# KaHIP/KaMinPar

Hardware: NVIDIA H100
Metric: lp_edges_per_second (higher is better)
Workload: dtype int32

## Files before the change

kaminpar_b200/csrc/kmp_lp.cu:

```cuda
#include <cuda_runtime.h>

#include <algorithm>
#include <chrono>
#include <cstdio>
#include <cstring>
#include <new>
#include <string>
#include <vector>

#include <cstdlib>
#include <dlfcn.h>
#include <nccl.h>
#include <cub/device/device_radix_sort.cuh>
#include <cub/device/device_scan.cuh>

#include "../../include/kaminpar_b200_contraction.h"
#include "../../include/kaminpar_b200_lp.h"
#include "lp_commit.cuh"
#include "lp_device.cuh"
#include "lp_lowgroup.cuh"
#include "lp_strict.cuh"
#include "lp_sweep.cuh"

using namespace kmp;
// ... 109 lines not shown
  uint32_t num_isolated = 0;

  DevBuf<uint32_t> order;
  std::vector<uint32_t> list_off;
  uint32_t max_list = 0;
  uint32_t lists_S = 0, lists_G = 0, lists_thr = 0;
  int lists_seed = 0;
  bool lists_valid = false;

  DevBuf<uint32_t> label, favored, communities;
  DevBuf<int32_t> weight, maxw, minw;
  DevBuf<uint8_t> active;
  DevBuf<uint32_t> mv_u, mv_t, cslot, slotmap;
  DevBuf<uint8_t> acc;
  DevBuf<int32_t> incoming, chist, hist, jmin, out_cur, out_delta, ohist, ojmin;
  DevBuf<uint32_t> ctr32;
  DevBuf<unsigned long long> ctr64;
  DevBuf<uint32_t> t4_table_off, t4_item_entry, t4_item_chunk, t4_sel_entry, t4_sel_piece, t4_sel_begin;
  DevBuf<uint32_t> t4_item_u, t4_item_beg, t4_item_deg;
  std::vector<uint32_t> t4_item_off, t4_sel_off;
  struct HubWave {
    uint32_t item_lo, item_hi, sel_lo, sel_hi;
  };
  std::vector<HubWave> t4_waves;
  std::vector<uint32_t> t4_wave_off;
  uint64_t hub_wave_slots = 1ull << 28;
  DevBuf<Cand> t4_part_best, t4_part_fav;
  uint64_t t4_max_slots = 0;
  uint64_t t4_max_wave_edges = 0;
  uint32_t hub_bucket_cap = kBucketCap, hub_sel_limit = 0;
  DevBuf<unsigned long long> hub_tab;
  DevBuf<uint32_t> hub_cursor;
  DevBuf<HubOverflow> hub_ovf;
  uint32_t mover_cap = 0;
  uint32_t cur_subround = 0;
  uint32_t cur_sg = 0;
  DevBuf<uint8_t> sort_keys_in, sort_keys_out;
  DevBuf<uint32_t> sort_vals_in;
  DevBuf<unsigned char> cub_tmp;
  DevBuf<unsigned long long> pairs_a, pairs_b;
  DevBuf<int32_t> ct_vals_a, ct_vals_b;
  DevBuf<uint32_t> ct_flags, ct_rank, ct_cl;
  DevBuf<unsigned long long> ct_counter;
  bool slot_state_clean = false;

  bool graph_sorted = false;
  bool strict_seeded = false;
  DevBuf<int32_t> st_slot, st_ent_val, st_slot2, st_ent2_val, st_concurrent;
  DevBuf<uint32_t> st_ent_key, st_ent2_key, st_used, st_second, st_tie_best, st_tie_fav, st_chunks, st_sub_perm,
      st_match, st_buckets;
  DevBuf<kmp_strict::Rng> st_rng;
  DevBuf<kmp_strict::Stats> st_stats;

  uint32_t call_counter = 0;
  uint64_t kernel_launches = 0, sweep_launches = 0;
  uint32_t pull_rounds = 0, push_rounds = 0;
  uint32_t rank = 0, world = 1;
  ncclComm_t comm = nullptr;
  DevBuf<uint32_t> dist_send, dist_recv;
  uint32_t *direct_send = nullptr;
  uint32_t direct_cap = 0;
  DevBuf<unsigned> grid_bar;
  int fused_blocks = 0;
  int fused_blocks_refine = 0;
  uint32_t low_blocks[2][2][2] = {};
  uint32_t team_grid[2][2][2][4] = {};
// ... 311 lines not shown
  const uint64_t b = (threads_needed + block - 1) / block;
  return static_cast<uint32_t>(std::max<uint64_t>(1, std::min<uint64_t>(b, max_blocks)));
}
inline uint32_t capped(const kmp_lp_handle *h, uint32_t blocks) {
  return h->grid_cap != 0 && blocks > h->grid_cap ? h->grid_cap : blocks;
}

constexpr int team_size_index(int T) { return T == 32 ? 0 : T == 128 ? 1 : T == 512 ? 2 : 3; }
template <int SLOTS, int TEAMS, bool V16> constexpr size_t team_smem() {
  return static_cast<size_t>(SLOTS) * TEAMS * (V16 ? 6 : 8);
}

template <int MODE, bool EW, bool P64, int T, int SLOTS, int TEAMS, bool V16 = false>
void launch_team(kmp_lp_handle *h, const SweepArgs &a) {
  const uint32_t want = (a.list_size + TEAMS - 1) / TEAMS;
  const uint32_t blocks = capped(h, std::max<uint32_t>(1, std::min<uint32_t>(want, h->team_grid[MODE][EW][P64][team_size_index(T)])));
  sweep_team<MODE, EW, P64, T, SLOTS, TEAMS, V16><<<blocks, T * TEAMS, team_smem<SLOTS, TEAMS, V16>(), h->sweep_stream>>>(a);
}

template <int MODE, bool EW, bool P64, int T, int SLOTS, int TEAMS, bool V16 = false>
bool configure_team(kmp_lp_handle *h, int sms) {
  const auto kernel = sweep_team<MODE, EW, P64, T, SLOTS, TEAMS, V16>;
  constexpr size_t smem = team_smem<SLOTS, TEAMS, V16>();
  int per_sm = 0;
  if (cudaFuncSetAttribute(kernel, cudaFuncAttributeMaxDynamicSharedMemorySize, static_cast<int>(smem)) != cudaSuccess ||
      cudaOccupancyMaxActiveBlocksPerMultiprocessor(&per_sm, kernel, T * TEAMS, smem) != cudaSuccess || per_sm < 1) {
    return false;
  }
  h->team_grid[MODE][EW][P64][team_size_index(T)] = static_cast<uint32_t>(sms * per_sm);
  return true;
}

template <int MODE, bool EW, bool P64> bool configure_team_kernels(kmp_lp_handle *h, int sms) {
  cudaFuncSetAttribute(sweep_hub_scatter<MODE, EW, P64>, cudaFuncAttributeMaxDynamicSharedMemorySize, kHubScatterSmem);
  bool ok = configure_team<MODE, EW, P64, 32, 512, 8, !EW>(h, sms) && configure_team<MODE, EW, P64, 128, 2048, 4>(h, sms) &&
            configure_team<MODE, EW, P64, 512, 8192, 1>(h, sms);
  if constexpr (EW) {
    ok = ok && configure_team<MODE, EW, P64, 1024, 16384, 1>(h, sms);
  } else {
    ok = ok && configure_team<MODE, EW, P64, 1024, 32768, 1, true>(h, sms);
  }
  return ok;
}

template <int MODE, bool EW, bool P64> cudaError_t launch_sweep_t(kmp_lp_handle *h, int tier, const SweepArgs &a) {
  if (a.list_size == 0) {
    return cudaSuccess;
  }
  const uint32_t tgrid = capped(h, grid_for(a.list_size, 256));
  switch (tier) {
  case 0:
    sweep_thread<MODE, EW, P64, 8><<<tgrid, 256, 0, h->sweep_stream>>>(a);
    break;
  case 1:
    sweep_thread<MODE, EW, P64, 16><<<tgrid, 256, 0, h->sweep_stream>>>(a);
    break;
  case 2:
    sweep_thread<MODE, EW, P64, 32><<<tgrid, 256, 0, h->sweep_stream>>>(a);
    break;
  case 3:
    launch_team<MODE, EW, P64, 32, 512, 8, !EW>(h, a);
    break;
  case 4:
    launch_team<MODE, EW, P64, 128, 2048, 4>(h, a);
    break;
  case 5:
    launch_team<MODE, EW, P64, 512, 8192, 1>(h, a);
    break;
  case 6:
    if constexpr (EW) {
      launch_team<MODE, EW, P64, 1024, 16384, 1>(h, a);
    } else {
      launch_team<MODE, EW, P64, 1024, 32768, 1, true>(h, a);
    }
    break;
  default: {
    HubArgs hb{};
    const uint32_t s_idx = h->cur_subround;
    const uint32_t S = h->lists_S;
    const uint32_t first = h->list_off[kHubTier * S + s_idx] - h->list_off[kHubTier * S];
    hb.table_off = h->t4_table_off.p + first;
    hb.g_tab = h->hub_tab.p;
    hb.cursor = h->hub_cursor.p;
    hb.ovf = h->hub_ovf.p;
    hb.ovf_cap = static_cast<uint32_t>(std::min<uint64_t>(h->t4_max_wave_edges, 0xFFFFFFFFull));
    hb.bucket_cap = h->hub_bucket_cap;
    hb.sel_limit = h->hub_sel_limit;
    hb.stage_adjncy = h->adjncy_16b ? 1u : 0u;
    hb.rank = h->rank;
    hb.world = h->world;
    hb.sel_begin = h->t4_sel_begin.p + first;
    hb.hit = h->t4_hit.p + first;
    for (uint32_t w = h->t4_wave_off[s_idx]; w < h->t4_wave_off[s_idx + 1]; ++w) {
      const kmp_lp_handle::HubWave &wv = h->t4_waves[w];
      hb.item_entry = h->t4_item_entry.p + wv.item_lo;
      hb.item_chunk = h->t4_item_chunk.p + wv.item_lo;
      hb.item_u = h->t4_item_u.p + wv.item_lo;
      hb.item_beg = h->t4_item_beg.p + wv.item_lo;
      hb.item_deg = h->t4_item_deg.p + wv.item_lo;
      hb.num_items = wv.item_hi - wv.item_lo;
      hb.queue = h->ctr32.p + 64 + w;
      hb.ovf_count = h->ctr32.p + 512 + w;
      sweep_hub_scatter<MODE, EW, P64><<<capped(h, std::min<uint32_t>(hb.num_items, kSMs * 4)), kHubThreads, kHubScatterSmem, h->sweep_stream>>>(a, hb, h->m);
      hb.sel_entry = h->t4_sel_entry.p + wv.sel_lo;
      hb.sel_piece = h->t4_sel_piece.p + wv.sel_lo;
      hb.num_sel_items = wv.sel_hi - wv.sel_lo;
      hb.part_best = h->t4_part_best.p + (wv.sel_lo - h->t4_sel_off[s_idx]);
      hb.part_fav = h->t4_part_fav.p + (wv.sel_lo - h->t4_sel_off[s_idx]);
      sweep_hub_select<MODE><<<capped(h, std::min<uint32_t>((hb.num_sel_items + kSelWarps - 1) / kSelWarps, kSMs * 6)), kSelWarps * 32, 0, h->sweep_stream>>>(a, hb);
      h->kernel_launches += 2;
    }
    hb.part_best = h->t4_part_best.p;
    hb.part_fav = h->t4_part_fav.p;
    sweep_hub_final<MODE><<<capped(h, grid_for(static_cast<uint64_t>(a.list_size) * 32, 256)), 256, 0, h->sweep_stream>>>(a, hb);
    break;
  }
  }
  return cudaGetLastError();
}

int timed_begin(kmp_lp_handle *h, int tag, cudaStream_t st = nullptr) {
  if (!h->timing) {
    return -1;
  }
  if (st == nullptr) {
    st = h->stream;
  }
  if (h->sweep_events_used == h->sweep_events.size()) {
    cudaEvent_t x, y;
    cudaEventCreate(&x);
    cudaEventCreate(&y);
    h->sweep_events.emplace_back(x, y);
    h->sweep_event_group.push_back(0);
  }
  const int idx = static_cast<int>(h->sweep_events_used++);
  h->sweep_event_group[idx] = tag;
  cudaEventRecord(h->sweep_events[idx].first, st);
  return idx;
}
void timed_end(kmp_lp_handle *h, int idx, cudaStream_t st = nullptr) {
  if (idx >= 0) {
    cudaEventRecord(h->sweep_events[idx].second, st == nullptr ? h->stream : st);
  }
// ... 91 lines not shown
                                             h->sort_vals_in.p, h->order.p, static_cast<int>(n), 0, 8, h->stream));
  }
  std::vector<uint32_t> hist(512);
  KMP_CUDA(cudaMemcpyAsync(hist.data(), h->ctr32.p, 512 * sizeof(uint32_t), cudaMemcpyDeviceToHost, h->stream));
  KMP_CUDA(cudaStreamSynchronize(h->stream));
  tc.lap("lists: keys + sort (sync)");
  h->list_off.assign(nkeys + 1, 0);
  for (uint32_t kx = 0; kx < nkeys; ++kx) {
    h->list_off[kx + 1] = h->list_off[kx] + hist[kx];
  }
  auto lsize = [&](uint32_t tier, uint32_t sr) { return hist[tier * S + sr]; };
  h->max_list = 0;
  h->mover_cap = 1;
  for (uint32_t sr = 0; sr < S; ++sr) {
    for (int g = 0; g < kNumGroups; ++g) {
      uint32_t tot = 0;
      for (int t = first_tier_of_group(g); t <= last_tier_of_group(g); ++t) {
        tot += lsize(static_cast<uint32_t>(t), sr);
      }
      h->mover_cap = std::max(h->mover_cap, tot);
    }
  }
  KMP_CUDA(h->queue.ensure(static_cast<size_t>(kNumTiers) * kNumGroups * S));
  h->max_list = h->mover_cap;
  h->max_degree = hist[300];
  {
    const uint32_t t4_begin = h->list_off[kHubTier * S], t4_end = h->list_off[(kHubTier + 1) * S];
    const uint32_t t4_cnt = t4_end - t4_begin;
    h->t4_item_off.assign(S + 1, 0);
    h->t4_wave_off.assign(S + 1, 0);
    h->t4_waves.clear();
    h->t4_max_slots = 0;
    h->t4_max_wave_edges = 0;
    if (t4_cnt > 0) {
      DevBuf<uint32_t> &d_deg = h->t4_tmp_deg, &d_beg = h->t4_tmp_beg, &d_ids = h->t4_tmp_ids;
      KMP_CUDA(d_deg.ensure(t4_cnt));
      KMP_CUDA(d_beg.ensure(t4_cnt));
      KMP_CUDA(d_ids.ensure(t4_cnt));
      k_gather_degrees<<<grid_for(t4_cnt, 256), 256, 0, h->stream>>>(t4_cnt, h->order.p + t4_begin, h->xadj, d_deg.p,
                                                                      d_beg.p, d_ids.p);
      std::vector<uint32_t> vbeg(t4_cnt), vids(t4_cnt), iu, ibeg, ideg;
      KMP_CUDA(cudaMemcpyAsync(vbeg.data(), d_beg.p, t4_cnt * sizeof(uint32_t), cudaMemcpyDeviceToHost, h->stream));
      KMP_CUDA(cudaMemcpyAsync(vids.data(), d_ids.p, t4_cnt * sizeof(uint32_t), cudaMemcpyDeviceToHost, h->stream));
      std::vector<uint32_t> deg(t4_cnt), toff(t4_cnt), sbeg(t4_cnt), ient, ichk, sent, spiece;
      h->t4_sel_off.assign(S + 1, 0);
      size_t max_sel = 0;
      KMP_CUDA(cudaMemcpyAsync(deg.data(), d_deg.p, t4_cnt * sizeof(uint32_t), cudaMemcpyDeviceToHost, h->stream));
      KMP_CUDA(cudaStreamSynchronize(h->stream));
      uint64_t wave_slots = h->hub_wave_slots;
      {
        uint64_t total = 0;
        for (uint32_t i = 0; i < t4_cnt; ++i) {
          total += static_cast<uint64_t>(hub_buckets(deg[i])) * kBucketCap;
        }
        wave_slots = std::max<uint64_t>(wave_slots, total / (kMaxHubWaves / 2 - S) + 1);
      }
      for (uint32_t sr = 0; sr < S; ++sr) {
        const uint32_t lo = h->list_off[kHubTier * S + sr] - t4_begin, hi = h->list_off[kHubTier * S + sr + 1] - t4_begin;
        uint64_t slots = 0, wave_edges = 0;
        kmp_lp_handle::HubWave wave{static_cast<uint32_t>(ient.size()), 0, static_cast<uint32_t>(sent.size()), 0};
        auto close_wave = [&]() {
          wave.item_hi = static_cast<uint32_t>(ient.size());
          wave.sel_hi = static_cast<uint32_t>(sent.size());
          if (wave.item_hi > wave.item_lo) {
            h->t4_waves.push_back(wave);
          }
// ... 9 lines not shown
          const uint64_t cap = static_cast<uint64_t>(buckets) * kBucketCap;
          if (slots > 0 && slots + cap > wave_slots) {
            close_wave();
          }
          if ((slots + cap) / kBucketCap > 0xFFFFFFFFull) {
            return fail(KMP_ERR_UNSUPPORTED, "high-degree buckets of one wave exceed 2^32");
          }
          toff[i] = static_cast<uint32_t>(slots / kBucketCap);
          slots += cap;
          wave_edges += deg[i];
          const uint32_t chunks = (deg[i] + kChunkEdges - 1) / kChunkEdges;
          for (uint32_t c = 0; c < chunks; ++c) {
            ient.push_back(i - lo);
            ichk.push_back(c);
            iu.push_back(vids[i]);
            ibeg.push_back(vbeg[i]);
            ideg.push_back(deg[i]);
          }
          sbeg[i] = static_cast<uint32_t>(sent.size() - h->t4_sel_off[sr]);
          for (uint32_t c = 0; c < buckets; ++c) {
            sent.push_back(i - lo);
            spiece.push_back(c);
          }
        }
        close_wave();
        h->t4_wave_off[sr + 1] = static_cast<uint32_t>(h->t4_waves.size());
        h->t4_sel_off[sr + 1] = static_cast<uint32_t>(sent.size());
        max_sel = std::max<size_t>(max_sel, sent.size() - h->t4_sel_off[sr]);
        h->t4_item_off[sr + 1] = static_cast<uint32_t>(ient.size());
      }
      if (h->t4_waves.size() > kMaxHubWaves) {
        return fail(KMP_ERR_UNSUPPORTED, "too many high-degree table waves (raise KMP_HUB_WAVE_SLOTS)");
      }
      KMP_CUDA(h->t4_table_off.ensure(t4_cnt));
      KMP_CUDA(h->t4_hit.ensure(t4_cnt));
      KMP_CUDA(cudaMemsetAsync(h->t4_hit.p, 0, static_cast<size_t>(t4_cnt) * 4, h->stream));
      KMP_CUDA(h->t4_item_entry.ensure(ient.size()));
      KMP_CUDA(h->t4_item_chunk.ensure(ichk.size()));
      KMP_CUDA(cudaMemcpyAsync(h->t4_table_off.p, toff.data(), t4_cnt * 4, cudaMemcpyHostToDevice, h->stream));
      KMP_CUDA(cudaMemcpyAsync(h->t4_item_entry.p, ient.data(), ient.size() * 4, cudaMemcpyHostToDevice, h->stream));
      KMP_CUDA(cudaMemcpyAsync(h->t4_item_chunk.p, ichk.data(), ichk.size() * 4, cudaMemcpyHostToDevice, h->stream));
      KMP_CUDA(h->t4_item_u.ensure(iu.size()));
      KMP_CUDA(h->t4_item_beg.ensure(iu.size()));
      KMP_CUDA(h->t4_item_deg.ensure(iu.size()));
      KMP_CUDA(cudaMemcpyAsync(h->t4_item_u.p, iu.data(), iu.size() * 4, cudaMemcpyHostToDevice, h->stream));
      KMP_CUDA(cudaMemcpyAsync(h->t4_item_beg.p, ibeg.data(), iu.size() * 4, cudaMemcpyHostToDevice, h->stream));
      KMP_CUDA(cudaMemcpyAsync(h->t4_item_deg.p, ideg.data(), iu.size() * 4, cudaMemcpyHostToDevice, h->stream));
      KMP_CUDA(h->t4_sel_entry.ensure(sent.size()));
      KMP_CUDA(h->t4_sel_piece.ensure(spiece.size()));
      KMP_CUDA(h->t4_sel_begin.ensure(t4_cnt));
      KMP_CUDA(h->t4_part_best.ensure(max_sel));
      KMP_CUDA(h->t4_part_fav.ensure(max_sel));
      KMP_CUDA(cudaMemcpyAsync(h->t4_sel_entry.p, sent.data(), sent.size() * 4, cudaMemcpyHostToDevice, h->stream));
      KMP_CUDA(cudaMemcpyAsync(h->t4_sel_piece.p, spiece.data(), spiece.size() * 4, cudaMemcpyHostToDevice, h->stream));
      KMP_CUDA(cudaMemcpyAsync(h->t4_sel_begin.p, sbeg.data(), t4_cnt * 4, cudaMemcpyHostToDevice, h->stream));
      KMP_CUDA(cudaStreamSynchronize(h->stream));
    }
  }
  tc.lap("lists: hub metadata");
  h->lists_S = S;
  h->lists_G = h->cfg.sync_granule_log2;
  h->lists_thr = h->cfg.large_degree_threshold;
  h->lists_seed = h->cfg.seed;
  h->lists_valid = true;
  tc.lap("lists: done");
  return KMP_OK;
}

int ensure_scratch(kmp_lp_handle *h, int mode, uint32_t num_labels) {
  const size_t cap = std::max<uint32_t>(h->mover_cap, 1);
  KMP_CUDA(h->mv_u.ensure(cap));
  KMP_CUDA(h->mv_t.ensure(cap));
  KMP_CUDA(h->acc.ensure(cap));
  KMP_CUDA(h->ctr32.ensure(kCtr32Size));
  KMP_CUDA(h->ctr64.ensure(kCtrSize));
  KMP_CUDA(h->active.ensure(h->n));
  if (mode == 0) {
    KMP_CUDA(h->cslot.ensure(cap));
    const bool fresh = h->incoming.cap < h->n || h->slotmap.cap < h->n || h->chist.cap < cap * kLadderLevels;
    KMP_CUDA(h->incoming.ensure(h->n));
    KMP_CUDA(h->slotmap.ensure(h->n));
    KMP_CUDA(h->chist.ensure(cap * kLadderLevels));
    if (fresh || !h->slot_state_clean) {
      KMP_CUDA(cudaMemsetAsync(h->incoming.p, 0, h->incoming.cap * sizeof(int32_t), h->stream));
      KMP_CUDA(cudaMemsetAsync(h->slotmap.p, 0xFF, h->slotmap.cap * sizeof(uint32_t), h->stream));
      KMP_CUDA(cudaMemsetAsync(h->chist.p, 0, h->chist.cap * sizeof(int32_t), h->stream));
      h->slot_state_clean = true;
    }
  } else {
    const size_t kk = std::max<uint32_t>(num_labels, 1);
    KMP_CUDA(h->hist.ensure(kk * kLadderLevels));
    KMP_CUDA(h->ohist.ensure(kk * kLadderLevels));
    KMP_CUDA(h->jmin.ensure(kk));
    KMP_CUDA(h->ojmin.ensure(kk));
    KMP_CUDA(h->out_cur.ensure(kk));
    KMP_CUDA(h->out_delta.ensure(kk));
    KMP_CUDA(cudaMemsetAsync(h->hist.p, 0, kk * kLadderLevels * sizeof(int32_t), h->stream));
    KMP_CUDA(cudaMemsetAsync(h->ohist.p, 0, kk * kLadderLevels * sizeof(int32_t), h->stream));
  }
  if (h->t4_max_slots > 0) {
    KMP_CUDA(h->hub_tab.ensure(h->t4_max_slots));
    KMP_CUDA(h->hub_cursor.ensure(h->t4_max_slots / kBucketCap));
    KMP_CUDA(h->hub_ovf.ensure(std::max<uint64_t>(h->t4_max_wave_edges, 1)));
    KMP_CUDA(cudaGetLastError());
  }
  (void)num_labels;
  return KMP_OK;
}

struct RunCtx {
  int mode;
  uint32_t num_labels;
  int32_t max_cluster_weight;
  bool has_min;
  bool has_comm;
};

SweepArgs make_sweep_args(kmp_lp_handle *h, const RunCtx &rc) {
  SweepArgs a{};
  a.xadj = h->xadj;
  a.adjncy = h->adjncy;
  a.vwgt = h->vwgt;
  a.adjwgt = h->adjwgt;
  a.label = h->label.p;
  a.labg = h->labg.p;
  a.pull = false;
  a.window = make_window(0, 0);
  a.queue = h->queue.p;
  a.weight = h->weight.p;
  a.max_w = rc.mode == 1 ? h->maxw.p : nullptr;
  a.min_w = rc.has_min ? h->minw.p : nullptr;
  a.communities = rc.has_comm ? h->communities.p : nullptr;
  a.active = h->active.p;
// ... 1339 lines not shown
}

int kmp_lp_free_scratch(kmp_lp_handle *h) {
  if (h == nullptr) {
    return KMP_OK;
  }
  cudaSetDevice(h->device);
  cudaStreamSynchronize(h->stream);
  h->label.release();
  h->favored.release();
  h->communities.release();
  h->weight.release();
  h->maxw.release();
  h->minw.release();
  h->active.release();
  h->mv_u.release();
  h->mv_t.release();
  h->cslot.release();
  h->slotmap.release();
  h->acc.release();
  h->incoming.release();
  h->chist.release();
  h->hist.release();
  h->jmin.release();
  h->out_cur.release();
  h->out_delta.release();
  h->ohist.release();
  h->ojmin.release();
  h->ctr32.release();
  h->ctr64.release();
  h->hub_tab.release();
  h->hub_cursor.release();
  h->hub_ovf.release();
  h->labg.release();
  h->sort_keys_in.release();
  h->sort_keys_out.release();
  h->sort_vals_in.release();
  h->t4_tmp_deg.release();
  h->t4_tmp_beg.release();
  h->t4_tmp_ids.release();
  h->cub_tmp.release();
  h->pairs_a.release();
  h->pairs_b.release();
  h->ct_vals_a.release();
  h->ct_vals_b.release();
  h->ct_flags.release();
  h->ct_rank.release();
  h->ct_cl.release();
  h->ct_counter.release();
  for (DevBuf<uint32_t> *b : {&h->bal_cand, &h->bal_under, &h->bal_ctr32, &h->bal_target, &h->bal_lists, &h->bal_sv_a,
                              &h->bal_sv_b, &h->bal_blk}) {
    b->release();
  }
  for (DevBuf<int32_t> *b : {&h->bal_over, &h->bal_pbw, &h->bal_wt, &h->bal_prefix}) {
    b->release();
  }
  h->bal_flag.release();
  h->bal_key.release();
  h->bal_ctrl.release();
  h->bal_sk_a.release();
  h->bal_sk_b.release();
  h->ubal_deficit.release();
  h->ubal_tmask.release();
  {
    cudaMemPool_t pool = kmp_private_pool(h->device);
    if (pool != nullptr) {
// ... 304 lines not shown
```

kaminpar_b200/csrc/lp_sweep.cuh:

```cuda
#pragma once

#include "lp_device.cuh"
#include "lp_sortnet.cuh"

namespace kmp {

template <int MODE>
__device__ __forceinline__ void emit_proposal(const SweepArgs &a, uint32_t idx, uint32_t u, uint32_t target,
                                              int32_t uw) {
  a.mv_u[idx] = u;
  a.mv_t[idx] = target;
  if (!a.accumulate) {
    return;
  }
  if (MODE == 0) {
    atomicAdd(&a.incoming[target], uw);
  } else {
    const uint32_t lvl = ladder_level(bijective32(u, a.base_commit));
    atomicAdd(&a.hist[target * kLadderLevels + lvl], uw);
  }
}

__device__ __forceinline__ void block_count_flush(const SweepArgs &a, unsigned long long edges,
                                                  unsigned long long nodes) {
// ... 555 lines not shown

struct HubOverflow {
  uint32_t bucket;
  uint32_t key;
  int32_t rating;
  uint32_t pad;
};

struct HubArgs {
  const uint32_t *__restrict__ item_entry;
  const uint32_t *__restrict__ item_chunk;
  const uint32_t *__restrict__ item_u;
  const uint32_t *__restrict__ item_beg;
  const uint32_t *__restrict__ item_deg;
  uint32_t num_items;
  const uint32_t *__restrict__ table_off;
  unsigned long long *__restrict__ g_tab;
  uint32_t *__restrict__ cursor;
  HubOverflow *__restrict__ ovf;
  uint32_t *__restrict__ ovf_count;
  uint32_t ovf_cap;
  uint32_t bucket_cap;
  uint32_t sel_limit;
  uint32_t stage_adjncy;
  const uint32_t *__restrict__ sel_entry;
  const uint32_t *__restrict__ sel_piece;
  uint32_t num_sel_items;
  const uint32_t *__restrict__ sel_begin;
  Cand *__restrict__ part_best;
  Cand *__restrict__ part_fav;
  uint32_t rank, world;
  uint32_t *__restrict__ queue;
  uint32_t *__restrict__ hit;
};

__host__ __device__ __forceinline__ uint32_t hub_buckets(uint32_t full_degree) {
  const uint32_t need = (full_degree + kBucketTargetFill - 1) / kBucketTargetFill;
  uint32_t p = 1;
  while (p < need) {
    p <<= 1;
  }
  return p;
}

__device__ __forceinline__ uint32_t smem_u32(const void *p) {
  return static_cast<uint32_t>(__cvta_generic_to_shared(p));
}
__device__ __forceinline__ void mbar_init(uint64_t *bar, uint32_t count) {
  asm volatile("mbarrier.init.shared::cta.b64 [%0], %1;" ::"r"(smem_u32(bar)), "r"(count) : "memory");
}
__device__ __forceinline__ void mbar_arrive_expect_tx(uint64_t *bar, uint32_t bytes) {
  asm volatile("mbarrier.arrive.expect_tx.shared::cta.b64 _, [%0], %1;" ::"r"(smem_u32(bar)), "r"(bytes) : "memory");
}
__device__ __forceinline__ void mbar_wait(uint64_t *bar, uint32_t parity) {
  asm volatile(
      "{\n"
      ".reg .pred p;\n"
      "WAIT_LOOP:\n"
      "mbarrier.try_wait.parity.shared::cta.b64 p, [%0], %1;\n"
      "@p bra DONE;\n"
      "bra WAIT_LOOP;\n"
      "DONE:\n"
      "}\n" ::"r"(smem_u32(bar)),
      "r"(parity)
      : "memory");
}
// ... 180 lines not shown
          kk[j] = keys[s];
          rr[j] = vals[s];
          if (kk[j] != kEmpty) {
            keys[s] = kEmpty;
            vals[s] = 0;
          }
        }
#pragma unroll
        for (int j = 0; j < B; ++j) {
          bb[j] = bucket0 + (lowbias32(kk[j]) & pmask);
          pos[j] = kk[j] != kEmpty ? atomicAdd(&hb.cursor[bb[j]], 1u) : 0u;
        }
#pragma unroll
        for (int j = 0; j < B; ++j) {
          if (kk[j] != kEmpty) {
            if (pos[j] < hb.bucket_cap) {
              hb.g_tab[static_cast<size_t>(bb[j]) * kBucketCap + pos[j]] =
                  (static_cast<unsigned long long>(kk[j]) << 32) | static_cast<uint32_t>(rr[j]);
            } else {
              const uint32_t o = atomicAdd(hb.ovf_count, 1u);
              if (o < hb.ovf_cap) {
                hb.ovf[o] = HubOverflow{bb[j], kk[j], rr[j], 0u};
              }
            }
          }
        }
      }
      __syncwarp();
    }
  }
}

template <int MODE> __global__ void __launch_bounds__(kSelWarps * 32) sweep_hub_select(const SweepArgs a, const HubArgs hb) {
  __shared__ uint32_t s_keys[kSelWarps][kSelTableSlots];
  __shared__ int32_t s_vals[kSelWarps][kSelTableSlots];
  __shared__ uint32_t s_claims_all[kSelWarps];
  const int lane = threadIdx.x & 31;
  const int wib = threadIdx.x >> 5;
  uint32_t *keys = s_keys[wib];
  int32_t *vals = s_vals[wib];
  uint32_t *s_claims = &s_claims_all[wib];
  for (uint32_t s = lane; s < kSelTableSlots; s += 32) {
    keys[s] = kEmpty;
    vals[s] = 0;
  }
  if (lane == 0) {
    *s_claims = 0;
  }
  __syncwarp();
  const uint32_t nwarps = gridDim.x * kSelWarps;
  for (uint32_t it = blockIdx.x * kSelWarps + wib; it < hb.num_sel_items; it += nwarps) {
    const uint32_t entry = hb.sel_entry[it];
    const uint32_t u = a.list[entry];
    Cand c = cand_none(), f = cand_none();
    const bool act = (entry % hb.world == hb.rank) && (a.active == nullptr || a.pull || a.active[u] != 0);
    const uint32_t b = hb.table_off[entry] + hb.sel_piece[it];
    const uint32_t appended = act ? __ldcg(&hb.cursor[b]) : 0u;
    if (appended != 0) {
      const uint32_t full_deg = a.xadj[u + 1] - a.xadj[u];
      const uint32_t pbits = 31 - __clz(static_cast<int>(hub_buckets(full_deg)));
      const uint32_t own = a.label[u];
      const int32_t uw = a.vwgt != nullptr ? a.vwgt[u] : 1;
      const int32_t own_w = a.weight[own];
      const bool store_fav = (MODE == 0) && (uw == own_w) && (own_w <= a.max_cluster_weight / 2);
      const uint32_t n_reg = appended < hb.bucket_cap ? appended : hb.bucket_cap;
      const uint32_t n_ovf = appended > hb.bucket_cap ? min(__ldcg(hb.ovf_count), hb.ovf_cap) : 0u;
      uint32_t tcap = pow2_ceil(2 * appended);
      tcap = tcap < 64 ? 64u : tcap > kSelTableSlots ? kSelTableSlots : tcap;
      const uint32_t tmask = tcap - 1;
      const uint32_t full_limit = tcap / 2 + tcap / 8;
      const uint32_t limit = (hb.sel_limit != 0 && hb.sel_limit < full_limit) ? hb.sel_limit : full_limit;
      const unsigned long long *reg = hb.g_tab + static_cast<size_t>(b) * kBucketCap;
      auto insert = [&](uint32_t key, int32_t r) {
        uint32_t slot = lowbias32(key ^ 0x9E3779B9u) & tmask;
        while (true) {
          const uint32_t prev = atomicCAS(&keys[slot], kEmpty, key);
          if (prev == kEmpty) {
            atomicAdd(s_claims, 1u);
          }
          if (prev == kEmpty || prev == key) {
            atomicAdd(&vals[slot], r);
            return;
          }
          slot = (slot + 1) & tmask;
        }
      };
      uint32_t K = 1;
      while (true) {
        c = cand_none();
        f = cand_none();
        bool overflowed = false;
        for (uint32_t cls = 0; cls < K && !overflowed; ++cls) {
          constexpr int B = 4;
          for (uint32_t i0 = 0; i0 < n_reg && !overflowed; i0 += 32 * B) {
            unsigned long long e[B];
#pragma unroll
            for (int j = 0; j < B; ++j) {
              const uint32_t i = i0 + j * 32 + lane;
              e[j] = i < n_reg ? __ldcs(reg + i) : ~0ull;
            }
#pragma unroll
            for (int j = 0; j < B; ++j) {
              const uint32_t key = static_cast<uint32_t>(e[j] >> 32);
              if (key != kEmpty && ((lowbias32(key) >> pbits) & (K - 1)) == cls) {
                insert(key, static_cast<int32_t>(static_cast<uint32_t>(e[j])));
              }
            }
            if (n_ovf != 0) {
              __syncwarp();
              overflowed = *s_claims > limit;
              __syncwarp();
            }
          }
          for (uint32_t i0 = 0; i0 < n_ovf && !overflowed; i0 += 32 * B) {
#pragma unroll
            for (int j = 0; j < B; ++j) {
              const uint32_t i = i0 + j * 32 + lane;
              if (i < n_ovf) {
                const HubOverflow o = hb.ovf[i];
                if (o.bucket == b && ((lowbias32(o.key) >> pbits) & (K - 1)) == cls) {
                  insert(o.key, o.rating);
                }
              }
            }
            __syncwarp();
            overflowed = *s_claims > limit;
            __syncwarp();
          }
          __syncwarp();
          bool lazy_done = false;
          if (MODE == 0 && K == 1 && !overflowed) {
            Cand ct = cand_none();
            for (uint32_t s = lane; s < tcap; s += 32) {
              const uint32_t kx = keys[s];
              if (kx != kEmpty) {
                const int32_t r = vals[s];
                if (r >= ct.gain && r > 0) {
                  const Cand x{r, 0, tie_hash(a.base_tie, u, kx), kx};
                  if (cand_better<0>(x, ct)) {
                    ct = x;
                  }
                }
                if (store_fav && r >= f.gain && r > 0) {
                  const Cand y{r, 0, tie_hash(a.base_fav, u, kx), kx};
                  if (cand_better<0>(y, f)) {
                    f = y;
                  }
                }
              }
            }
            const Cand top = warp_argmax<0>(kFull, ct);
            bool top_ok = true;
            if (top.gain > 0) {
              top_ok = (a.weight[top.key] + uw <= a.max_cluster_weight) || (top.key == own);
              if (a.communities != nullptr) {
                top_ok = top_ok && (a.communities[top.key] == a.communities[own]);
              }
            }
            if (top_ok) {
              c = top;
              lazy_done = true;
            }
          }
          const bool evaluate = !overflowed && !lazy_done;
          for (uint32_t s0 = 0; s0 < tcap; s0 += 32 * B) {
            uint32_t kk[B];
            int32_t rr[B], ww[B];
#pragma unroll
            for (int j = 0; j < B; ++j) {
              const uint32_t s = s0 + j * 32 + lane;
              kk[j] = s < tcap ? keys[s] : kEmpty;
              rr[j] = kk[j] != kEmpty ? vals[s] : 0;
            }
#pragma unroll
            for (int j = 0; j < B; ++j) {
              ww[j] = (kk[j] != kEmpty && evaluate) ? a.weight[kk[j]] : 0;
            }
#pragma unroll
            for (int j = 0; j < B; ++j) {
              if (kk[j] != kEmpty) {
                const uint32_t s = s0 + j * 32 + lane;
                keys[s] = kEmpty;
                vals[s] = 0;
                if (evaluate) {
                  Cand ff;
                  const Cand cc = eval_candidate_w<MODE>(a, u, own, uw, own_w, kk[j], rr[j], ww[j],
                                                         store_fav && !(MODE == 0 && K == 1), ff);
                  if (cand_better<MODE>(cc, c)) {
                    c = cc;
                  }
                  if (MODE == 0 && cand_better<0>(ff, f)) {
                    f = ff;
                  }
                }
              }
            }
          }
          __syncwarp();
          if (lane == 0) {
            *s_claims = 0;
          }
          __syncwarp();
        }
        if (!overflowed) {
          break;
        }
        K <<= 1;
      }
      if (lane == 0) {
        hb.cursor[b] = 0;
      }
    }
    const Cand best = warp_argmax<MODE>(kFull, c);
    const Cand fav = (MODE == 0) ? warp_argmax<0>(kFull, f) : cand_none();
    if (lane == 0) {
      hb.part_best[it] = best;
      hb.part_fav[it] = fav;
    }
  }
}

template <int MODE> __global__ void __launch_bounds__(256) sweep_hub_final(const SweepArgs a, const HubArgs hb) {
  const int lane = threadIdx.x & 31;
  const uint32_t warp = (blockIdx.x * blockDim.x + threadIdx.x) >> 5;
  const uint32_t nwarps = (gridDim.x * blockDim.x) >> 5;
  unsigned long long edges = 0, nodes = 0;
  for (uint32_t i = warp; i < a.list_size; i += nwarps) {
    if (i % hb.world != hb.rank) {
      continue;
    }
    const uint32_t u = a.list[i];
    bool flag = true;
    if (a.active != nullptr) {
      int fl = 0, ht = 0;
      if (lane == 0) {
        fl = static_cast<int>(a.active[u]);
        if (a.pull) {
          ht = static_cast<int>(hb.hit[i]);
          hb.hit[i] = 0;
        }
      }
      fl = __shfl_sync(kFull, fl, 0);
      ht = __shfl_sync(kFull, ht, 0);
      flag = fl != 0;
      if (fl == 0 && ht == 0) {
        continue;
      }
    }
    const uint32_t full_deg = a.xadj[u + 1] - a.xadj[u];
    uint32_t deg = full_deg;
    if (deg > a.max_num_neighbors) {
      deg = a.max_num_neighbors;
    }
    const uint32_t own = a.label[u];
    const int32_t uw = a.vwgt != nullptr ? a.vwgt[u] : 1;
    const int32_t own_w = a.weight[own];
    const uint32_t pieces = hub_buckets(full_deg);
    const uint32_t first = hb.sel_begin[i];
    const bool store_fav = (MODE == 0) && (uw == own_w) && (own_w <= a.max_cluster_weight / 2);
    Cand c = cand_none(), f = cand_none();
    for (uint32_t q = lane; q < pieces; q += 32) {
      const Cand pb = hb.part_best[first + q];
      if (cand_better<MODE>(pb, c)) {
        c = pb;
      }
      if (MODE == 0) {
        const Cand pf = hb.part_fav[first + q];
        if (cand_better<0>(pf, f)) {
          f = pf;
        }
      }
    }
    const Cand best = warp_argmax<MODE>(kFull, c);
    const Cand fav = (MODE == 0) ? warp_argmax<0>(kFull, f) : cand_none();
    if (lane == 0) {
      edges += deg;
      nodes += 1;
      if (a.active != nullptr && flag) {
        a.active[u] = 0;
      }
      uint32_t target;
      if (finish_vertex<MODE>(a, u, own, store_fav, best, fav, target)) {
        const uint32_t idx = atomicAdd(a.mover_count, 1u);
        emit_proposal<MODE>(a, idx, u, target, uw);
      }
    }
  }
  block_count_flush(a, edges, nodes);
}

// ... 2 lines not shown
```

Before: 41.33 billion.

## Rate clusterer hub nodes via label gather and per-class shared-memory hashing

For the clustering mode, high-degree hub nodes are no longer scattered into global hash buckets and then selected per wave. Instead, one kernel gathers neighbor labels into a contiguous buffer. A 1024-thread block then rates each hash class of labels in a large shared-memory table, and splits the class further if the table overflows. Work items are ordered by descending degree. This removes the global atomic scatter, the bucket and overflow bookkeeping, and the per-wave launches. In exchange, every hub's degree is re-read once per class pass and an extra label buffer is allocated.

```diff
diff --git a/kaminpar_b200/csrc/kmp_lp.cu b/kaminpar_b200/csrc/kmp_lp.cu
--- a/kaminpar_b200/csrc/kmp_lp.cu
+++ b/kaminpar_b200/csrc/kmp_lp.cu
@@ -165,6 +165,10 @@
   DevBuf<unsigned long long> hub_tab;
   DevBuf<uint32_t> hub_cursor;
   DevBuf<HubOverflow> hub_ovf;
+  DevBuf<uint32_t> t4_lab_off, t4_rate_begin, t4_rate_entry, t4_rate_cls;
+  std::vector<uint32_t> t4_rate_off;
+  uint64_t t4_max_subround_edges = 0;
+  DevBuf<uint32_t> hub_lab;
   uint32_t mover_cap = 0;
   uint32_t cur_subround = 0;
   uint32_t cur_sg = 0;
@@ -542,7 +546,13 @@
 }
 
 template <int MODE, bool EW, bool P64> bool configure_team_kernels(kmp_lp_handle *h, int sms) {
-  cudaFuncSetAttribute(sweep_hub_scatter<MODE, EW, P64>, cudaFuncAttributeMaxDynamicSharedMemorySize, kHubScatterSmem);
+  if constexpr (MODE == 0) {
+    if (cudaFuncSetAttribute(sweep_hub_rate<EW>, cudaFuncAttributeMaxDynamicSharedMemorySize, rate_smem<EW>()) != cudaSuccess) {
+      return false;
+    }
+  } else {
+    cudaFuncSetAttribute(sweep_hub_scatter<MODE, EW, P64>, cudaFuncAttributeMaxDynamicSharedMemorySize, kHubScatterSmem);
+  }
   bool ok = configure_team<MODE, EW, P64, 32, 512, 8, !EW>(h, sms) && configure_team<MODE, EW, P64, 128, 2048, 4>(h, sms) &&
             configure_team<MODE, EW, P64, 512, 8192, 1>(h, sms);
   if constexpr (EW) {
@@ -589,36 +599,59 @@
     const uint32_t s_idx = h->cur_subround;
     const uint32_t S = h->lists_S;
     const uint32_t first = h->list_off[kHubTier * S + s_idx] - h->list_off[kHubTier * S];
-    hb.table_off = h->t4_table_off.p + first;
-    hb.g_tab = h->hub_tab.p;
-    hb.cursor = h->hub_cursor.p;
-    hb.ovf = h->hub_ovf.p;
-    hb.ovf_cap = static_cast<uint32_t>(std::min<uint64_t>(h->t4_max_wave_edges, 0xFFFFFFFFull));
-    hb.bucket_cap = h->hub_bucket_cap;
     hb.sel_limit = h->hub_sel_limit;
-    hb.stage_adjncy = h->adjncy_16b ? 1u : 0u;
     hb.rank = h->rank;
     hb.world = h->world;
-    hb.sel_begin = h->t4_sel_begin.p + first;
     hb.hit = h->t4_hit.p + first;
-    for (uint32_t w = h->t4_wave_off[s_idx]; w < h->t4_wave_off[s_idx + 1]; ++w) {
-      const kmp_lp_handle::HubWave &wv = h->t4_waves[w];
-      hb.item_entry = h->t4_item_entry.p + wv.item_lo;
-      hb.item_chunk = h->t4_item_chunk.p + wv.item_lo;
-      hb.item_u = h->t4_item_u.p + wv.item_lo;
-      hb.item_beg = h->t4_item_beg.p + wv.item_lo;
-      hb.item_deg = h->t4_item_deg.p + wv.item_lo;
-      hb.num_items = wv.item_hi - wv.item_lo;
-      hb.queue = h->ctr32.p + 64 + w;
-      hb.ovf_count = h->ctr32.p + 512 + w;
-      sweep_hub_scatter<MODE, EW, P64><<<capped(h, std::min<uint32_t>(hb.num_items, kSMs * 4)), kHubThreads, kHubScatterSmem, h->sweep_stream>>>(a, hb, h->m);
-      hb.sel_entry = h->t4_sel_entry.p + wv.sel_lo;
-      hb.sel_piece = h->t4_sel_piece.p + wv.sel_lo;
-      hb.num_sel_items = wv.sel_hi - wv.sel_lo;
-      hb.part_best = h->t4_part_best.p + (wv.sel_lo - h->t4_sel_off[s_idx]);
-      hb.part_fav = h->t4_part_fav.p + (wv.sel_lo - h->t4_sel_off[s_idx]);
-      sweep_hub_select<MODE><<<capped(h, std::min<uint32_t>((hb.num_sel_items + kSelWarps - 1) / kSelWarps, kSMs * 6)), kSelWarps * 32, 0, h->sweep_stream>>>(a, hb);
+    if constexpr (MODE == 0) {
+      const uint32_t ilo = h->t4_item_off[s_idx], ihi = h->t4_item_off[s_idx + 1];
+      hb.item_entry = h->t4_item_entry.p + ilo;
+      hb.item_chunk = h->t4_item_chunk.p + ilo;
+      hb.item_u = h->t4_item_u.p + ilo;
+      hb.item_beg = h->t4_item_beg.p + ilo;
+      hb.item_deg = h->t4_item_deg.p + ilo;
+      hb.num_items = ihi - ilo;
+      hb.lab = h->hub_lab.p;
+      hb.lab_off = h->t4_lab_off.p + first;
+      sweep_hub_gather<P64><<<capped(h, std::min<uint32_t>(hb.num_items, kSMs * 8)), 256, 0, h->sweep_stream>>>(a, hb);
+      const uint32_t rlo = h->t4_rate_off[s_idx], rhi = h->t4_rate_off[s_idx + 1];
+      hb.item_entry = h->t4_rate_entry.p + rlo;
+      hb.item_cls = h->t4_rate_cls.p + rlo;
+      hb.num_items = rhi - rlo;
+      hb.sel_begin = h->t4_rate_begin.p + first;
+      hb.part_best = h->t4_part_best.p;
+      hb.part_fav = h->t4_part_fav.p;
+      hb.queue = h->ctr32.p + 64 + s_idx;
+      sweep_hub_rate<EW><<<capped(h, std::min<uint32_t>(hb.num_items, kSMs)), kRateThreads, rate_smem<EW>(), h->sweep_stream>>>(a, hb);
       h->kernel_launches += 2;
+    } else {
+      hb.table_off = h->t4_table_off.p + first;
+      hb.g_tab = h->hub_tab.p;
+      hb.cursor = h->hub_cursor.p;
+      hb.ovf = h->hub_ovf.p;
+      hb.ovf_cap = static_cast<uint32_t>(std::min<uint64_t>(h->t4_max_wave_edges, 0xFFFFFFFFull));
+      hb.bucket_cap = h->hub_bucket_cap;
+      hb.stage_adjncy = h->adjncy_16b ? 1u : 0u;
+      hb.sel_begin = h->t4_sel_begin.p + first;
+      for (uint32_t w = h->t4_wave_off[s_idx]; w < h->t4_wave_off[s_idx + 1]; ++w) {
+        const kmp_lp_handle::HubWave &wv = h->t4_waves[w];
+        hb.item_entry = h->t4_item_entry.p + wv.item_lo;
+        hb.item_chunk = h->t4_item_chunk.p + wv.item_lo;
+        hb.item_u = h->t4_item_u.p + wv.item_lo;
+        hb.item_beg = h->t4_item_beg.p + wv.item_lo;
+        hb.item_deg = h->t4_item_deg.p + wv.item_lo;
+        hb.num_items = wv.item_hi - wv.item_lo;
+        hb.queue = h->ctr32.p + 64 + w;
+        hb.ovf_count = h->ctr32.p + 512 + w;
+        sweep_hub_scatter<MODE, EW, P64><<<capped(h, std::min<uint32_t>(hb.num_items, kSMs * 4)), kHubThreads, kHubScatterSmem, h->sweep_stream>>>(a, hb, h->m);
+        hb.sel_entry = h->t4_sel_entry.p + wv.sel_lo;
+        hb.sel_piece = h->t4_sel_piece.p + wv.sel_lo;
+        hb.num_sel_items = wv.sel_hi - wv.sel_lo;
+        hb.part_best = h->t4_part_best.p + (wv.sel_lo - h->t4_sel_off[s_idx]);
+        hb.part_fav = h->t4_part_fav.p + (wv.sel_lo - h->t4_sel_off[s_idx]);
+        sweep_hub_select<MODE><<<capped(h, std::min<uint32_t>((hb.num_sel_items + kSelWarps - 1) / kSelWarps, kSMs * 6)), kSelWarps * 32, 0, h->sweep_stream>>>(a, hb);
+        h->kernel_launches += 2;
+      }
     }
     hb.part_best = h->t4_part_best.p;
     hb.part_fav = h->t4_part_fav.p;
@@ -776,6 +809,7 @@
     h->t4_waves.clear();
     h->t4_max_slots = 0;
     h->t4_max_wave_edges = 0;
+    h->t4_max_subround_edges = 0;
     if (t4_cnt > 0) {
       DevBuf<uint32_t> &d_deg = h->t4_tmp_deg, &d_beg = h->t4_tmp_beg, &d_ids = h->t4_tmp_ids;
       KMP_CUDA(d_deg.ensure(t4_cnt));
@@ -851,6 +885,41 @@
       if (h->t4_waves.size() > kMaxHubWaves) {
         return fail(KMP_ERR_UNSUPPORTED, "too many high-degree table waves (raise KMP_HUB_WAVE_SLOTS)");
       }
+      std::vector<uint32_t> loff(t4_cnt), rbeg(t4_cnt), rent, rcls, ord;
+      h->t4_rate_off.assign(S + 1, 0);
+      size_t max_rate = 0;
+      for (uint32_t sr = 0; sr < S; ++sr) {
+        const uint32_t lo = h->list_off[kHubTier * S + sr] - t4_begin, hi = h->list_off[kHubTier * S + sr + 1] - t4_begin;
+        uint64_t edges = 0;
+        uint32_t res = 0;
+        ord.clear();
+        for (uint32_t i = lo; i < hi; ++i) {
+          loff[i] = static_cast<uint32_t>(edges);
+          edges += deg[i];
+          rbeg[i] = res;
+          res += hub_classes(deg[i]);
+          ord.push_back(i);
+        }
+        std::stable_sort(ord.begin(), ord.end(), [&](uint32_t x, uint32_t y) { return deg[x] > deg[y]; });
+        for (const uint32_t i : ord) {
+          for (uint32_t c = 0; c < hub_classes(deg[i]); ++c) {
+            rent.push_back(i - lo);
+            rcls.push_back(c);
+          }
+        }
+        h->t4_rate_off[sr + 1] = static_cast<uint32_t>(rent.size());
+        max_rate = std::max<size_t>(max_rate, res);
+        h->t4_max_subround_edges = std::max(h->t4_max_subround_edges, edges);
+      }
+      max_sel = std::max(max_sel, max_rate);
+      KMP_CUDA(h->t4_lab_off.ensure(t4_cnt));
+      KMP_CUDA(h->t4_rate_begin.ensure(t4_cnt));
+      KMP_CUDA(h->t4_rate_entry.ensure(rent.size()));
+      KMP_CUDA(h->t4_rate_cls.ensure(rcls.size()));
+      KMP_CUDA(cudaMemcpyAsync(h->t4_lab_off.p, loff.data(), t4_cnt * 4, cudaMemcpyHostToDevice, h->stream));
+      KMP_CUDA(cudaMemcpyAsync(h->t4_rate_begin.p, rbeg.data(), t4_cnt * 4, cudaMemcpyHostToDevice, h->stream));
+      KMP_CUDA(cudaMemcpyAsync(h->t4_rate_entry.p, rent.data(), rent.size() * 4, cudaMemcpyHostToDevice, h->stream));
+      KMP_CUDA(cudaMemcpyAsync(h->t4_rate_cls.p, rcls.data(), rcls.size() * 4, cudaMemcpyHostToDevice, h->stream));
       KMP_CUDA(h->t4_table_off.ensure(t4_cnt));
       KMP_CUDA(h->t4_hit.ensure(t4_cnt));
       KMP_CUDA(cudaMemsetAsync(h->t4_hit.p, 0, static_cast<size_t>(t4_cnt) * 4, h->stream));
@@ -917,7 +986,10 @@
     KMP_CUDA(cudaMemsetAsync(h->hist.p, 0, kk * kLadderLevels * sizeof(int32_t), h->stream));
     KMP_CUDA(cudaMemsetAsync(h->ohist.p, 0, kk * kLadderLevels * sizeof(int32_t), h->stream));
   }
-  if (h->t4_max_slots > 0) {
+  if (mode == 0 && h->t4_max_subround_edges > 0) {
+    KMP_CUDA(h->hub_lab.ensure(h->t4_max_subround_edges));
+  }
+  if (mode == 1 && h->t4_max_slots > 0) {
     KMP_CUDA(h->hub_tab.ensure(h->t4_max_slots));
     KMP_CUDA(h->hub_cursor.ensure(h->t4_max_slots / kBucketCap));
     KMP_CUDA(h->hub_ovf.ensure(std::max<uint64_t>(h->t4_max_wave_edges, 1)));
@@ -2323,6 +2395,7 @@
   h->hub_tab.release();
   h->hub_cursor.release();
   h->hub_ovf.release();
+  h->hub_lab.release();
   h->labg.release();
   h->sort_keys_in.release();
   h->sort_keys_out.release();
diff --git a/kaminpar_b200/csrc/lp_sweep.cuh b/kaminpar_b200/csrc/lp_sweep.cuh
--- a/kaminpar_b200/csrc/lp_sweep.cuh
+++ b/kaminpar_b200/csrc/lp_sweep.cuh
@@ -611,6 +611,9 @@
   uint32_t rank, world;
   uint32_t *__restrict__ queue;
   uint32_t *__restrict__ hit;
+  uint32_t *__restrict__ lab;
+  const uint32_t *__restrict__ lab_off;
+  const uint32_t *__restrict__ item_cls;
 };
 
 __host__ __device__ __forceinline__ uint32_t hub_buckets(uint32_t full_degree) {
@@ -857,6 +860,7 @@
 }
 
 template <int MODE> __global__ void __launch_bounds__(kSelWarps * 32) sweep_hub_select(const SweepArgs a, const HubArgs hb) {
+  static_assert(MODE == 1, "the clusterer rates its hubs with sweep_hub_rate");
   __shared__ uint32_t s_keys[kSelWarps][kSelTableSlots];
   __shared__ int32_t s_vals[kSelWarps][kSelTableSlots];
   __shared__ uint32_t s_claims_all[kSelWarps];
@@ -877,7 +881,7 @@
   for (uint32_t it = blockIdx.x * kSelWarps + wib; it < hb.num_sel_items; it += nwarps) {
     const uint32_t entry = hb.sel_entry[it];
     const uint32_t u = a.list[entry];
-    Cand c = cand_none(), f = cand_none();
+    Cand c = cand_none();
     const bool act = (entry % hb.world == hb.rank) && (a.active == nullptr || a.pull || a.active[u] != 0);
     const uint32_t b = hb.table_off[entry] + hb.sel_piece[it];
     const uint32_t appended = act ? __ldcg(&hb.cursor[b]) : 0u;
@@ -887,7 +891,6 @@
       const uint32_t own = a.label[u];
       const int32_t uw = a.vwgt != nullptr ? a.vwgt[u] : 1;
       const int32_t own_w = a.weight[own];
-      const bool store_fav = (MODE == 0) && (uw == own_w) && (own_w <= a.max_cluster_weight / 2);
       const uint32_t n_reg = appended < hb.bucket_cap ? appended : hb.bucket_cap;
       const uint32_t n_ovf = appended > hb.bucket_cap ? min(__ldcg(hb.ovf_count), hb.ovf_cap) : 0u;
       uint32_t tcap = pow2_ceil(2 * appended);
@@ -913,7 +916,6 @@
       uint32_t K = 1;
       while (true) {
         c = cand_none();
-        f = cand_none();
         bool overflowed = false;
         for (uint32_t cls = 0; cls < K && !overflowed; ++cls) {
           constexpr int B = 4;
@@ -953,41 +955,7 @@
             __syncwarp();
           }
           __syncwarp();
-          bool lazy_done = false;
-          if (MODE == 0 && K == 1 && !overflowed) {
-            Cand ct = cand_none();
-            for (uint32_t s = lane; s < tcap; s += 32) {
-              const uint32_t kx = keys[s];
-              if (kx != kEmpty) {
-                const int32_t r = vals[s];
-                if (r >= ct.gain && r > 0) {
-                  const Cand x{r, 0, tie_hash(a.base_tie, u, kx), kx};
-                  if (cand_better<0>(x, ct)) {
-                    ct = x;
-                  }
-                }
-                if (store_fav && r >= f.gain && r > 0) {
-                  const Cand y{r, 0, tie_hash(a.base_fav, u, kx), kx};
-                  if (cand_better<0>(y, f)) {
-                    f = y;
-                  }
-                }
-              }
-            }
-            const Cand top = warp_argmax<0>(kFull, ct);
-            bool top_ok = true;
-            if (top.gain > 0) {
-              top_ok = (a.weight[top.key] + uw <= a.max_cluster_weight) || (top.key == own);
-              if (a.communities != nullptr) {
-                top_ok = top_ok && (a.communities[top.key] == a.communities[own]);
-              }
-            }
-            if (top_ok) {
-              c = top;
-              lazy_done = true;
-            }
-          }
-          const bool evaluate = !overflowed && !lazy_done;
+          const bool evaluate = !overflowed;
           for (uint32_t s0 = 0; s0 < tcap; s0 += 32 * B) {
             uint32_t kk[B];
             int32_t rr[B], ww[B];
@@ -1009,13 +977,9 @@
                 vals[s] = 0;
                 if (evaluate) {
                   Cand ff;
-                  const Cand cc = eval_candidate_w<MODE>(a, u, own, uw, own_w, kk[j], rr[j], ww[j],
-                                                         store_fav && !(MODE == 0 && K == 1), ff);
-                  if (cand_better<MODE>(cc, c)) {
+                  const Cand cc = eval_candidate_w<1>(a, u, own, uw, own_w, kk[j], rr[j], ww[j], false, ff);
+                  if (cand_better<1>(cc, c)) {
                     c = cc;
-                  }
-                  if (MODE == 0 && cand_better<0>(ff, f)) {
-                    f = ff;
                   }
                 }
               }
@@ -1036,12 +1000,298 @@
         hb.cursor[b] = 0;
       }
     }
-    const Cand best = warp_argmax<MODE>(kFull, c);
-    const Cand fav = (MODE == 0) ? warp_argmax<0>(kFull, f) : cand_none();
+    const Cand best = warp_argmax<1>(kFull, c);
     if (lane == 0) {
       hb.part_best[it] = best;
-      hb.part_fav[it] = fav;
-    }
+    }
+  }
+}
+
+constexpr int kRateThreads = 1024;
+constexpr uint32_t kRateSlots = 16384;
+constexpr uint32_t kRateListCap = kRateSlots / 2;
+constexpr uint32_t kHubClassEdges = 8192;
+constexpr uint32_t kRateStage = 64;
+template <bool EW> constexpr int rate_smem() {
+  return static_cast<int>(kRateSlots * 8 + kRateListCap * 2 + (kRateThreads / 32) * kRateStage * (EW ? 8 : 4));
+}
+
+__host__ __device__ __forceinline__ uint32_t hub_classes(uint32_t full_degree) {
+  const uint32_t need = (full_degree + kHubClassEdges - 1) / kHubClassEdges;
+  uint32_t p = 1;
+  while (p < need) {
+    p <<= 1;
+  }
+  return p;
+}
+
+template <bool P64> __global__ void __launch_bounds__(256) sweep_hub_gather(const SweepArgs a, const HubArgs hb) {
+  constexpr int B = kChunkEdges / 256;
+  const int lane = threadIdx.x & 31;
+  for (uint32_t it = blockIdx.x; it < hb.num_items; it += gridDim.x) {
+    const uint32_t entry = hb.item_entry[it];
+    const uint32_t u = hb.item_u[it];
+    if (entry % hb.world != hb.rank || !(a.active == nullptr || a.pull || a.active[u] != 0)) {
+      continue;
+    }
+    const uint32_t deg = min(hb.item_deg[it], a.max_num_neighbors);
+    const uint32_t cbeg = hb.item_chunk[it] * kChunkEdges;
+    if (cbeg >= deg) {
+      continue;
+    }
+    const uint32_t cend = min(cbeg + kChunkEdges, deg);
+    const uint32_t *adj = a.adjncy + hb.item_beg[it];
+    uint32_t *out = hb.lab + hb.lab_off[entry];
+    uint32_t v[B];
+#pragma unroll
+    for (int j = 0; j < B; ++j) {
+      const uint32_t e = cbeg + j * 256 + threadIdx.x;
+      v[j] = e < cend ? adj[e] : kEmpty;
+    }
+    bool hit = false;
+#pragma unroll
+    for (int j = 0; j < B; ++j) {
+      if (v[j] != kEmpty) {
+        const typename LabG<P64>::word g = load_labg<P64>(a, v[j]);
+        hit = hit || stamp_hit(LabG<P64>::stamp(g), a.window);
+        out[cbeg + j * 256 + threadIdx.x] = LabG<P64>::label(g);
+      }
+    }
+    if (a.pull && __any_sync(kFull, hit) && lane == 0) {
+      atomicOr(&hb.hit[entry], 1u);
+    }
+  }
+}
+
+template <bool EW>
+__device__ __forceinline__ bool rate_insert(uint32_t *keys, int32_t *vals, uint16_t *list, uint32_t *s_claims,
+                                            uint32_t limit, uint32_t key, int32_t w, bool valid, int lane) {
+  uint32_t slot = 0;
+  bool claimed = false;
+  if (valid) {
+    slot = lowbias32(key ^ 0x9E3779B9u) & (kRateSlots - 1);
+    while (true) {
+      const uint32_t prev = atomicCAS(&keys[slot], kEmpty, key);
+      if (prev == kEmpty || prev == key) {
+        claimed = prev == kEmpty;
+        if (EW || !claimed) {
+          atomicAdd(&vals[slot], w);
+        }
+        break;
+      }
+      slot = (slot + 1) & (kRateSlots - 1);
+    }
+  }
+  const unsigned mask = __ballot_sync(kFull, claimed);
+  if (mask == 0) {
+    return false;
+  }
+  const uint32_t n = __popc(mask);
+  uint32_t base = 0;
+  if (lane == 0) {
+    base = atomicAdd(s_claims, n);
+  }
+  base = __shfl_sync(kFull, base, 0);
+  const uint32_t idx = base + __popc(mask & ((1u << lane) - 1u));
+  if (claimed && idx < kRateListCap) {
+    list[idx] = static_cast<uint16_t>(slot);
+  }
+  return base + n > limit;
+}
+
+template <bool EW> __global__ void __launch_bounds__(kRateThreads, 1) sweep_hub_rate(const SweepArgs a, const HubArgs hb) {
+  constexpr int T = kRateThreads;
+  constexpr int kWarps = T / 32;
+  constexpr int B = 8;
+  extern __shared__ __align__(16) unsigned char smem_raw[];
+  uint32_t *keys = reinterpret_cast<uint32_t *>(smem_raw);
+  int32_t *vals = reinterpret_cast<int32_t *>(smem_raw + sizeof(uint32_t) * kRateSlots);
+  uint32_t *stage_k = reinterpret_cast<uint32_t *>(smem_raw + 8 * kRateSlots);
+  int32_t *stage_w = reinterpret_cast<int32_t *>(stage_k + kWarps * kRateStage);
+  uint16_t *list = reinterpret_cast<uint16_t *>(stage_k + (EW ? 2 : 1) * kWarps * kRateStage);
+  __shared__ Cand s_red[kWarps];
+  __shared__ uint32_t s_item, s_claims;
+  const int tid = threadIdx.x;
+  const int lane = tid & 31;
+  const int wib = tid >> 5;
+  const unsigned below = (1u << lane) - 1u;
+  uint32_t *stk = stage_k + wib * kRateStage;
+  int32_t *stw = stage_w + wib * kRateStage;
+  for (uint32_t s = tid; s < kRateSlots; s += T) {
+    keys[s] = kEmpty;
+    vals[s] = 0;
+  }
+  const uint32_t limit = (hb.sel_limit != 0 && hb.sel_limit < kRateListCap) ? max(hb.sel_limit, 2u) : kRateListCap;
+  while (true) {
+    if (tid == 0) {
+      s_item = atomicAdd(hb.queue, 1u);
+    }
+    __syncthreads();
+    const uint32_t it = s_item;
+    if (it >= hb.num_items) {
+      break;
+    }
+    const uint32_t entry = hb.item_entry[it];
+    const uint32_t c0 = hb.item_cls[it];
+    const uint32_t u = a.list[entry];
+    if (entry % hb.world == hb.rank && (a.active == nullptr || a.pull || a.active[u] != 0)) {
+      const uint32_t beg = a.xadj[u];
+      const uint32_t full_deg = a.xadj[u + 1] - beg;
+      const uint32_t deg = min(full_deg, a.max_num_neighbors);
+      const uint32_t K0 = hub_classes(full_deg);
+      const uint32_t own = a.label[u];
+      const int32_t uw = a.vwgt != nullptr ? a.vwgt[u] : 1;
+      const int32_t own_w = a.weight[own];
+      const bool store_fav = (uw == own_w) && (own_w <= a.max_cluster_weight / 2);
+      const uint32_t *lab = hb.lab + hb.lab_off[entry];
+      Cand best = cand_none(), fav = cand_none();
+      uint32_t cls = c0, K = K0;
+      while (true) {
+        if (tid == 0) {
+          s_claims = 0;
+        }
+        __syncthreads();
+        bool wover = false;
+        uint32_t head = 0, pend = 0;
+        for (uint32_t e0 = wib * 32 * B; e0 < deg && !wover; e0 += T * B) {
+          uint32_t kb[B];
+#pragma unroll
+          for (int j = 0; j < B; ++j) {
+            const uint32_t e = e0 + j * 32 + lane;
+            kb[j] = e < deg ? __ldcg(lab + e) : kEmpty;
+          }
+#pragma unroll
+          for (int j = 0; j < B; ++j) {
+            if (!wover) {
+              const bool in = kb[j] != kEmpty && (lowbias32(kb[j]) & (K - 1)) == cls;
+              const unsigned m = __ballot_sync(kFull, in);
+              if (in) {
+                const uint32_t pos = (head + pend + __popc(m & below)) & (kRateStage - 1);
+                stk[pos] = kb[j];
+                if (EW) {
+                  stw[pos] = a.adjwgt[beg + e0 + j * 32 + lane];
+                }
+              }
+              pend += __popc(m);
+              if (pend >= 32) {
+                __syncwarp();
+                const uint32_t sl = (head + lane) & (kRateStage - 1);
+                wover = rate_insert<EW>(keys, vals, list, &s_claims, limit, stk[sl], EW ? stw[sl] : 1, true, lane);
+                __syncwarp();
+                head = (head + 32) & (kRateStage - 1);
+                pend -= 32;
+              }
+            }
+          }
+        }
+        if (!wover) {
+          __syncwarp();
+          const bool v = lane < pend;
+          const uint32_t sl = (head + lane) & (kRateStage - 1);
+          wover = rate_insert<EW>(keys, vals, list, &s_claims, limit, v ? stk[sl] : 0u, (EW && v) ? stw[sl] : 1, v, lane);
+        }
+        const bool over = __syncthreads_or(wover);
+        if (over) {
+          for (uint32_t s = tid; s < kRateSlots; s += T) {
+            keys[s] = kEmpty;
+            vals[s] = 0;
+          }
+          K <<= 1;
+          __syncthreads();
+          continue;
+        }
+        const uint32_t nc = s_claims;
+        Cand c = cand_none(), f = cand_none();
+        for (uint32_t l = tid; l < nc; l += T) {
+          const uint32_t s = list[l];
+          const uint32_t k = keys[s];
+          const int32_t r = vals[s] + (EW ? 0 : 1);
+          if (r > 0 && r >= c.gain) {
+            const Cand x{r, 0, tie_hash(a.base_tie, u, k), k};
+            if (cand_better<0>(x, c)) {
+              c = x;
+            }
+          }
+          if (store_fav && r > 0 && r >= f.gain) {
+            const Cand y{r, 0, tie_hash(a.base_fav, u, k), k};
+            if (cand_better<0>(y, f)) {
+              f = y;
+            }
+          }
+        }
+        Cand cb = team_argmax<0, T>(1, tid, c, s_red);
+        if (store_fav) {
+          const Cand cf = team_argmax<0, T>(1, tid, f, s_red);
+          if (cand_better<0>(cf, fav)) {
+            fav = cf;
+          }
+        }
+        bool top_ok = true;
+        if (cb.gain > 0) {
+          top_ok = (a.weight[cb.key] + uw <= a.max_cluster_weight) || (cb.key == own);
+          if (a.communities != nullptr) {
+            top_ok = top_ok && (a.communities[cb.key] == a.communities[own]);
+          }
+        }
+        if (!top_ok) {
+          Cand ce = cand_none();
+          for (uint32_t l0 = 0; l0 < nc; l0 += T * 4) {
+            uint32_t kk[4];
+            int32_t rr[4], ww[4];
+#pragma unroll
+            for (int j = 0; j < 4; ++j) {
+              const uint32_t l = l0 + j * T + tid;
+              const uint32_t s = l < nc ? list[l] : 0u;
+              kk[j] = l < nc ? keys[s] : kEmpty;
+              rr[j] = l < nc ? vals[s] + (EW ? 0 : 1) : 0;
+            }
+#pragma unroll
+            for (int j = 0; j < 4; ++j) {
+              ww[j] = kk[j] != kEmpty ? a.weight[kk[j]] : 0;
+            }
+#pragma unroll
+            for (int j = 0; j < 4; ++j) {
+              if (kk[j] != kEmpty) {
+                Cand ff;
+                const Cand cc = eval_candidate_w<0>(a, u, own, uw, own_w, kk[j], rr[j], ww[j], false, ff);
+                if (cand_better<0>(cc, ce)) {
+                  ce = cc;
+                }
+              }
+            }
+          }
+          cb = team_argmax<0, T>(1, tid, ce, s_red);
+        }
+        if (cand_better<0>(cb, best)) {
+          best = cb;
+        }
+        for (uint32_t l = tid; l < nc; l += T) {
+          const uint32_t s = list[l];
+          keys[s] = kEmpty;
+          vals[s] = 0;
+        }
+        __syncthreads();
+        bool done = true;
+        while (K > K0) {
+          const uint32_t half = K >> 1;
+          if ((cls & half) == 0) {
+            cls |= half;
+            done = false;
+            break;
+          }
+          cls &= ~half;
+          K = half;
+        }
+        if (done) {
+          break;
+        }
+      }
+      if (tid == 0) {
+        hb.part_best[hb.sel_begin[entry] + c0] = best;
+        hb.part_fav[hb.sel_begin[entry] + c0] = fav;
+      }
+    }
+    __syncthreads();
   }
 }
 
@@ -1080,7 +1330,7 @@
     const uint32_t own = a.label[u];
     const int32_t uw = a.vwgt != nullptr ? a.vwgt[u] : 1;
     const int32_t own_w = a.weight[own];
-    const uint32_t pieces = hub_buckets(full_deg);
+    const uint32_t pieces = MODE == 0 ? hub_classes(full_deg) : hub_buckets(full_deg);
     const uint32_t first = hb.sel_begin[i];
     const bool store_fav = (MODE == 0) && (uw == own_w) && (own_w <= a.max_cluster_weight / 2);
     Cand c = cand_none(), f = cand_none();
```

Result: faster. 43.60 billion, median of 6 (+5.5%).
